# openai/baselines

Hardware: NVIDIA H100
Metric: PPO2 learner env-steps/sec (higher is better)
Workload: dtype f16 operands / f32 accumulate (GAE f64 carry)

## Files before the change

### baselines_b200/csrc/common.cuh

```cuda
#pragma once
#include <cuda.h>
#include <cuda_fp16.h>
#include <cuda_runtime.h>
#include <stdint.h>

#include "../../include/b200rl.h"

namespace b200rl {

void set_last_error(const char* fmt, ...);

inline int check_launch(const char* what) {
  cudaError_t e = cudaGetLastError();
  if (e != cudaSuccess) {
    set_last_error("%s: %s", what, cudaGetErrorString(e));
    return B200RL_ERR_CUDA;
  }
  return B200RL_OK;
}

#define B200RL_REQUIRE(cond, ...)                 \
  do {                                            \
    if (!(cond)) {                                \
      ::b200rl::set_last_error(__VA_ARGS__);      \
      return B200RL_ERR_ARG;                      \
    }                                             \
  } while (0)

__host__ __device__ inline int ceil_div(int a, int b) { return (a + b - 1) / b; }
__host__ __device__ inline long long ceil_div_ll(long long a, long long b) { return (a + b - 1) / b; }

float* det_workspace(size_t floats, cudaStream_t stream);
int sum_partials(const float* ws, int parts, long long rows, int cols, float* out, long long ldo, cudaStream_t stream);
int device_num_sms();

#ifdef __CUDACC__
__device__ __forceinline__ uint32_t smem_u32(const void* p) {
  return static_cast<uint32_t>(__cvta_generic_to_shared(p));
}

__device__ __forceinline__ void mbar_init(uint64_t* bar, uint32_t count) {
  asm volatile("mbarrier.init.shared::cta.b64 [%0], %1;" ::"r"(smem_u32(bar)), "r"(count));
}
__device__ __forceinline__ void fence_barrier_init() {
  asm volatile("fence.mbarrier_init.release.cluster;" ::: "memory");
}
__device__ __forceinline__ void fence_proxy_async_smem() {
  asm volatile("fence.proxy.async.shared::cta;" ::: "memory");
}
__device__ __forceinline__ void mbar_arrive_expect_tx(uint64_t* bar, uint32_t bytes) {
  asm volatile("mbarrier.arrive.expect_tx.shared::cta.b64 _, [%0], %1;" ::"r"(smem_u32(bar)), "r"(bytes)
               : "memory");
}
__device__ __forceinline__ void mbar_arrive(uint64_t* bar) {
  asm volatile("mbarrier.arrive.shared::cta.b64 _, [%0];" ::"r"(smem_u32(bar)) : "memory");
}
static constexpr uint32_t MBAR_SUSPEND_NS = 20000;
__device__ __forceinline__ bool mbar_try_wait(uint64_t* bar, uint32_t parity) {
  uint32_t ok;
  asm volatile(
      "{\n\t.reg .pred p;\n\t"
      "mbarrier.try_wait.parity.shared::cta.b64 p, [%1], %2, %3;\n\t"
      "selp.u32 %0, 1, 0, p;\n\t}"
      : "=r"(ok)
      : "r"(smem_u32(bar)), "r"(parity), "r"(MBAR_SUSPEND_NS)
      : "memory");
  return ok != 0;
}
__device__ __forceinline__ void mbar_wait(uint64_t* bar, uint32_t parity) {
  while (!mbar_try_wait(bar, parity)) {
  }
}

__device__ __forceinline__ uint32_t cluster_ctarank() {
  uint32_t r;
  asm volatile("mov.u32 %0, %%cluster_ctarank;" : "=r"(r));
  return r;
}
__device__ __forceinline__ uint32_t cluster_nctarank() {
  uint32_t n;
  asm volatile("mov.u32 %0, %%cluster_nctarank;" : "=r"(n));
  return n;
}
__device__ __forceinline__ void cluster_sync() {
  asm volatile("barrier.cluster.arrive.release;\n\tbarrier.cluster.wait.acquire;" ::: "memory");
// ... 62 lines not shown
```

### baselines_b200/csrc/conv_shift.cu

```cuda
#include <stdlib.h>

#include <type_traits>

#include "common.cuh"
#include "tc_common.cuh"

namespace b200rl {

static constexpr int SH_BM = 128;
static constexpr int SH_CONSUMER_WARPS = 8;
static constexpr int SH_TMA_WARP = SH_CONSUMER_WARPS;
__host__ __device__ constexpr int sh_threads(bool u8) { return (SH_CONSUMER_WARPS + 1) * 32 + (u8 ? 256 : 0); }
static constexpr int SH_MAX_TAPS = 16;
__host__ __device__ constexpr int sh_arows(int KH) { return KH == 1 ? 160 : 144; }
__host__ __device__ constexpr int sh_stages(int KH) { return KH == 1 ? 6 : 4; }
static constexpr int SH_U8_STAGES = 12;
static constexpr int SH_U8_WRES_BYTES = 16 * 1024;
__host__ __device__ constexpr int sh_wgrad_krows(bool u8) { return u8 ? 128 : 64; }
__host__ __device__ constexpr int sh_wres_bytes(int KH, bool u8) {
  return u8 ? SH_U8_WRES_BYTES : KH == 1 ? 80 * 1024 : 64 * 1024;
}
static constexpr int SH_BAR_BYTES = 512;
__host__ __device__ constexpr int sh_mask_stage_bytes(int BN, bool DACT) { return DACT ? SH_BM * BN / 8 : 0; }
static constexpr int SH_EPI_WARP_BYTES = 16 * 64;
static constexpr int SH_EPI_BYTES = SH_CONSUMER_WARPS * SH_EPI_WARP_BYTES;
static constexpr int SH_WROWS_K = 96;
static constexpr int SH_WABYTES = SH_WROWS_K * 128;
__host__ __device__ constexpr int sh_wgrad_qw(int BN, int KH, bool u8) { return u8 ? 2 : BN == 32 ? 4 : KH == 1 ? 3 : 2; }

static constexpr int SH_ORDER_BAR = 2;
__device__ __forceinline__ void order_wait(int wg) {
  asm volatile("bar.sync %0, %1;" ::"r"(SH_ORDER_BAR + wg), "n"(SH_CONSUMER_WARPS * 32) : "memory");
}
__device__ __forceinline__ void order_pass(int wg) {
  asm volatile("bar.arrive %0, %1;" ::"r"(SH_ORDER_BAR + 1 - wg), "n"(SH_CONSUMER_WARPS * 32) : "memory");
}

struct AddrMap {
  int mode;
  long long sN, sY, sX;
  int Cq, s;
  int Cq_log2, s_log2;
};

__device__ __forceinline__ long long map_rowbase(const AddrMap& a, int n, int y, int x) {
  if (a.mode == 2) {
    const int sm = a.s - 1;
    return (long long)n * a.sN + (long long)(y >> a.s_log2) * a.sY + (long long)(x >> a.s_log2) * a.sX +
           ((((y & sm) << a.s_log2) + (x & sm)) << a.Cq_log2);
  }
  if (a.mode == 1) return (long long)n * a.sN + ((long long)y << a.s_log2) * a.sY + ((long long)x << a.s_log2) * a.sX;
  return (long long)n * a.sN + (long long)y * a.sY + (long long)x * a.sX;
}
__device__ __forceinline__ long long map_coloff(const AddrMap& a, int col) {
  if (a.mode == 1) {
    const int cls = col >> a.Cq_log2;
    return (long long)(cls >> a.s_log2) * a.sY + (long long)(cls & (a.s - 1)) * a.sX + (col & (a.Cq - 1));
  }
  return col;
}

struct FastDiv {
  uint32_t mul, sh, d;
  __device__ __forceinline__ uint32_t div(uint32_t n) const { return __umulhi(n, mul) >> sh; }
};
static FastDiv make_fastdiv(uint32_t d) {
  FastDiv f;
  f.d = d;
  uint32_t s = 0;
// ... 9 lines not shown
  const long long* idx;
  long long sample_bytes;
  int row_bytes;
  int y_bytes, x_bytes;
  FastDiv per, wg;
};

static constexpr int U8_WARPS = 8;

__device__ __forceinline__ void u8x16_to_f16(const uint4& q, uint4& lo, uint4& hi) {
  const uint32_t w[4] = {q.x, q.y, q.z, q.w};
  uint32_t o[8];
  const __half2 k1024 = __floats2half2_rn(1024.0f, 1024.0f);
#pragma unroll
  for (int i = 0; i < 4; ++i) {
    const uint32_t a = __byte_perm(w[i], 0x64646464u, 0x5140);
    const uint32_t b = __byte_perm(w[i], 0x64646464u, 0x5342);
    const __half2 ha = __hsub2(*reinterpret_cast<const __half2*>(&a), k1024);
    const __half2 hb = __hsub2(*reinterpret_cast<const __half2*>(&b), k1024);
    o[2 * i] = *reinterpret_cast<const uint32_t*>(&ha);
    o[2 * i + 1] = *reinterpret_cast<const uint32_t*>(&hb);
  }
  lo = make_uint4(o[0], o[1], o[2], o[3]);
  hi = make_uint4(o[4], o[5], o[6], o[7]);
}


__device__ __forceinline__ uint4 ldg_stream_v4(const void* p) {
  uint4 v;
  asm volatile("ld.global.nc.L1::no_allocate.v4.u32 {%0,%1,%2,%3}, [%4];"
               : "=r"(v.x), "=r"(v.y), "=r"(v.z), "=r"(v.w)
               : "l"(p));
  return v;
}
__device__ __forceinline__ void st_shared_v4(uint32_t addr, const uint4& v) {
  asm volatile("st.shared.v4.b32 [%0], {%1,%2,%3,%4};" ::"r"(addr), "r"(v.x), "r"(v.y), "r"(v.z), "r"(v.w) : "memory");
}

template <int TR, int STAGES>
struct U8Ring {
  static constexpr int UPT = TR / 32;
  static constexpr int ROWS = STAGES * TR + 32;
  static constexpr int BYTES = ROWS * 128;
  static_assert(TR % 32 == 0 && BYTES % 1024 == 0, "ring keeps the 1024 B swizzle atoms aligned");
};

__device__ __forceinline__ long long u8_lookup(const U8Src& u, long long row_start, int unit, int total, long long M,
                                               int lane) {
  const long long m = row_start + (long long)unit * 32 + lane;
  if (unit >= total || m < 0 || m >= M) return -1;
  const uint32_t n = u.per.div((uint32_t)m);
  return u.idx ? __ldg(u.idx + n) : (long long)n;
}
__device__ __forceinline__ void u8_load(const U8Src& u, long long row_start, int unit, long long sb, int lane,
                                        uint4 (&q)[4]) {
  if (sb >= 0) {
    const uint32_t mm = (uint32_t)(row_start + (long long)unit * 32 + lane);
    const uint32_t rem = mm - u.per.div(mm) * u.per.d;
    const uint32_t Y = u.wg.div(rem), X = rem - Y * u.wg.d;
    const uint8_t* src = u.x + sb * u.sample_bytes + (long long)(Y * (uint32_t)u.y_bytes + X * (uint32_t)u.x_bytes);
#pragma unroll
    for (int dy = 0; dy < 4; ++dy) q[dy] = ldg_stream_v4(src + (long long)dy * u.row_bytes);
  } else {
#pragma unroll
    for (int dy = 0; dy < 4; ++dy) q[dy] = make_uint4(0u, 0u, 0u, 0u);
  }
}

template <int TR, int STAGES, int D>
// ... 38 lines not shown
        }
        fence_proxy_async_smem();
        __syncwarp();
        if (lane == 0) {
          if (tile < ntiles) mbar_arrive(&full_bar[s]);
          if (ub == 0) mbar_arrive(&head_bar[s]);
        }
        u8_load(u, row_start, uc + RND, sb[d], lane, q[d]);
        sb[d] = u8_lookup(u, row_start, uc + 2 * RND, total, M, lane);
      }
    }
  }
}

struct ShiftParams {
  U8Src u8;
  FastDiv fwg, fhg;
  long long M;
  int Hg, Wg;
  int N;
  int taps;
  int shift[SH_MAX_TAPS];
  int min_shift;
  int vy, vx;
  __half* out;
  AddrMap omap;
  uint16_t* bits_out;
  const uint16_t* saved_bits;
  const float* bias;
  int act, dact;
  float alpha;
  int num_tiles;
};

__device__ __forceinline__ void stmatrix_x4(uint32_t addr, const uint32_t (&r)[4]) {
  asm volatile("stmatrix.sync.aligned.m8n8.x4.shared.b16 [%0], {%1, %2, %3, %4};" ::"r"(addr), "r"(r[0]), "r"(r[1]),
               "r"(r[2]), "r"(r[3])
               : "memory");
}
__device__ __forceinline__ uint4 ld_shared_v4(uint32_t addr) {
  uint4 v;
  asm volatile("ld.shared.v4.b32 {%0,%1,%2,%3}, [%4];" : "=r"(v.x), "=r"(v.y), "=r"(v.z), "=r"(v.w) : "r"(addr) : "memory");
  return v;
}
__device__ __forceinline__ void st_global_v4(void* p, const uint4& v) {
  asm volatile("st.global.v4.b32 [%0], {%1,%2,%3,%4};" ::"l"(p), "r"(v.x), "r"(v.y), "r"(v.z), "r"(v.w) : "memory");
}
__device__ __forceinline__ uint32_t h2_bits(__half2 h) { return *reinterpret_cast<const uint32_t*>(&h); }
__device__ __forceinline__ uint32_t mask_pair(uint32_t b8, int k) {
  const uint32_t b = b8 >> (2 * k);
  return ((b & 1u) | ((b & 2u) << 15)) * 0xffffu;
}

template <int BN, int KH, bool DACT, bool U8>
__global__ void __launch_bounds__(sh_threads(U8), 1)
conv_shift_fwd_kernel(const __grid_constant__ CUtensorMap tmX, const __grid_constant__ CUtensorMap tmW,
                      const __grid_constant__ ShiftParams p) {
  constexpr int SH_ABYTES = sh_arows(KH) * 128;
  constexpr int STAGE_BYTES = KH * SH_ABYTES;
  constexpr int STAGES = U8 ? SH_U8_STAGES : sh_stages(KH);
  using Ring = U8Ring<SH_BM, STAGES>;
  constexpr bool PINGPONG = !(BN == 128 && !DACT);
  constexpr int MH = PINGPONG ? 2 : 1;
  static_assert(PINGPONG || !U8, "the uint8 ring's release rule assumes ping-pong");
  constexpr int A_PITCH = U8 ? SH_BM * 128 : STAGE_BYTES;
  constexpr int A_TOTAL = U8 ? Ring::BYTES : STAGES * STAGE_BYTES;
  extern __shared__ uint8_t smem_raw[];
  uint8_t* smem = reinterpret_cast<uint8_t*>((reinterpret_cast<uintptr_t>(smem_raw) + 1023) & ~uintptr_t(1023));
  uint8_t* wres = smem + A_TOTAL;
  uint64_t* bars = reinterpret_cast<uint64_t*>(wres + sh_wres_bytes(KH, U8));
  uint64_t* full_bar = bars;
  uint64_t* empty_bar = bars + STAGES;
  uint64_t* w_bar = bars + 2 * STAGES;
  uint64_t* head_bar = bars + 2 * STAGES + 1;
  static_assert((3 * STAGES + 1) * 8 <= SH_BAR_BYTES, "barrier block");
  constexpr int MASK_STAGE = sh_mask_stage_bytes(BN, DACT);
  uint8_t* smask = reinterpret_cast<uint8_t*>(bars) + SH_BAR_BYTES;
  uint8_t* sepi = smask + STAGES * MASK_STAGE;

  __shared__ float s_bias[BN];
  const int warp = threadIdx.x >> 5, lane = threadIdx.x & 31;
  constexpr int w_sub = BN * 128;
  if (threadIdx.x < BN) s_bias[threadIdx.x] = (p.bias && (int)threadIdx.x < p.N) ? p.bias[threadIdx.x] : 0.0f;
  if (threadIdx.x == 0) {
    for (int s = 0; s < STAGES; ++s) {
// ... 640 lines not shown
```

### baselines_b200/csrc/gemm_wgmma.cu

```cuda
#include <stdarg.h>
#include <stdio.h>
#include <stdlib.h>

#include <map>
#include <mutex>

#include "common.cuh"
#include "tc_common.cuh"

namespace b200rl {

static constexpr int BM = 128;
static constexpr int BK = 64;
static constexpr int MMA_K = 16;
static constexpr int CONSUMER_WARPS = 8;
static constexpr int NUM_THREADS = CONSUMER_WARPS * 32 + 32;


struct ConvCoords {
  int OW, OH;
  int stride_w, stride_h;
  int lower_w, lower_h;
  int S, taps;
};

struct ShuffleOut {
  int H, W, C, s;
};

struct GemmParams {
  int M, N, K;
  int m_tiles, n_tiles, splits, kb_per_split, kb_total;
  void* C;
  long long ldc;
  const float* bias;
  const __half* saved;
  const uint16_t* saved_bits;
  long long ld_saved;
  float alpha;
  int mode, act;
  ConvCoords cv;
  ShuffleOut sh;
  bool vec32;
  int rm_C, rm_OW, rm_Wg;
  float* ws;
};

template <int BN>
struct Cfg {
  static constexpr int A_BYTES = BM * BK * 2;
  static constexpr int B_BYTES = BN * BK * 2;
  static constexpr int STAGE_BYTES = A_BYTES + B_BYTES;
  static constexpr int STAGES_RAW = (196 * 1024) / STAGE_BYTES;
  static constexpr int STAGES = STAGES_RAW > 8 ? 8 : STAGES_RAW;
  static constexpr int SMEM_BYTES = STAGES * STAGE_BYTES + 1024  + 256 ;
};

static constexpr int BRES_STAGES = 7;
static constexpr int BRES_B_BYTES = 80 * 1024;

__device__ __forceinline__ void gemm_epi_pair(const GemmParams& p, int mode, int split, int row, int col, float v0,
                                              float v1, bool two) {
  if (mode == MODE_F32_ATOMIC) {
    if (p.ws) {
      float* w = p.ws + ((long long)split * p.M + row) * p.N + col;
      w[0] = v0;
      if (two) w[1] = v1;
      return;
    }
    float* out = reinterpret_cast<float*>(p.C) + (long long)row * p.ldc + col;
    atomicAdd(out, v0);
    if (two) atomicAdd(out + 1, v1);
    return;
  }
  if (mode == MODE_F32_STORE) {
    float* out = reinterpret_cast<float*>(p.C) + (long long)row * p.ldc + col;
    out[0] = v0 + (p.bias ? p.bias[col] : 0.0f);
    if (two) out[1] = v1 + (p.bias ? p.bias[col + 1] : 0.0f);
    return;
  }
  __half* C = reinterpret_cast<__half*>(p.C);
  if (mode == MODE_F16_SHUFFLE) {
    const int cls = col / p.sh.C, c = col % p.sh.C;
    const int j = row % p.cv.OW, t3 = row / p.cv.OW;
    const int i = t3 % p.cv.OH, n = t3 / p.cv.OH;
    const int y = p.sh.s * i + cls / p.sh.s, x = p.sh.s * j + cls % p.sh.s;
    if (y < p.sh.H && x < p.sh.W) {
      const long long o = (((long long)n * p.sh.H + y) * p.sh.W + x) * p.sh.C + c;
      if (p.saved) {
        v0 *= act_grad_from_saved(__half2float(p.saved[o]), p.act);
        v1 *= act_grad_from_saved(__half2float(p.saved[o + 1]), p.act);
      }
// ... 31 lines not shown
  } else {
    out[0] = __float2half_rn(v0);
    if (two) out[1] = __float2half_rn(v1);
  }
}

template <int BN, int CPT, bool MN_MAJOR, bool IM2COL, bool BRES, int TMODE>
__global__ void __launch_bounds__(NUM_THREADS, 1)
gemm_wgmma_kernel(const __grid_constant__ CUtensorMap tmA, const __grid_constant__ CUtensorMap tmB,
                  const GemmParams p) {
  using C_ = Cfg<BN>;
  static_assert(!BRES || (IM2COL && !MN_MAJOR), "resident weights: K-major implicit conv only");
  constexpr int STAGES = BRES ? BRES_STAGES : C_::STAGES;
  constexpr int STAGE_BYTES = BRES ? C_::A_BYTES : C_::STAGE_BYTES;
  constexpr int BROWB = MN_MAJOR ? (BN >= 64 ? 128 : BN * 2) : 0;
  constexpr uint32_t LAYOUT_B = sdesc_layout(BROWB);
  constexpr int BCHUNKS = (BN >= 64) ? BN / 64 : 1;
  constexpr int TPS = BK / CPT;
  constexpr int ROWB = CPT * 2;
  constexpr uint32_t LAYOUT_A = sdesc_layout(ROWB);
  constexpr int A_SUB = BM * ROWB;
  constexpr int B_SUB = BN * ROWB;
  constexpr int A_CHUNK = BK * ROWB;
  constexpr int MCH = BM / CPT;
  extern __shared__ uint8_t smem_raw[];
  uint8_t* smem = reinterpret_cast<uint8_t*>((reinterpret_cast<uintptr_t>(smem_raw) + 1023) & ~uintptr_t(1023));
  uint8_t* bres = smem + STAGES * STAGE_BYTES;
  constexpr int ZT_BYTES = (IM2COL && !MN_MAJOR) ? B_SUB : 0;
  uint8_t* zero_tile = bres + (BRES ? BRES_B_BYTES : 0);
  uint64_t* bars = reinterpret_cast<uint64_t*>(zero_tile + ZT_BYTES);
  uint64_t* full_bar = bars;
  uint64_t* empty_bar = bars + STAGES;
  uint64_t* bres_bar = bars + 2 * STAGES;

  const int warp = threadIdx.x >> 5;
  const int lane = threadIdx.x & 31;
  const int total_work = p.m_tiles * p.n_tiles * p.splits;

  if (threadIdx.x == 0) {
    for (int s = 0; s < STAGES; ++s) {
      mbar_init(&full_bar[s], 1);
      mbar_init(&empty_bar[s], CONSUMER_WARPS);
    }
    mbar_init(bres_bar, 1);
    fence_barrier_init();
  }
  __syncthreads();

  if (warp == CONSUMER_WARPS) {
    if (elect_one()) {
      tma_prefetch_desc(&tmA);
      tma_prefetch_desc(&tmB);
      if (BRES) {
        mbar_arrive_expect_tx(bres_bar, (uint32_t)p.cv.taps * B_SUB);
        for (int g = 0; g < p.cv.taps; ++g) tma_load_2d(bres + g * B_SUB, &tmB, bres_bar, g * CPT, 0);
      }
    }
    __syncwarp();
    int s = 0;
    uint32_t ph = 0;
    for (int work = blockIdx.x; work < total_work; work += gridDim.x) {
      const int n_tile = work % p.n_tiles;
      const int t2 = work / p.n_tiles;
      const int m_tile = t2 % p.m_tiles;
      const int split = t2 / p.m_tiles;
      const int kb0 = split * p.kb_per_split;
      const int kb1 = min(kb0 + p.kb_per_split, p.kb_total);
      int cw = 0, ch = 0, cn = 0;
      if (IM2COL && !MN_MAJOR) {
        const int m0 = m_tile * BM;
        const int q = m0 % p.cv.OW, t3 = m0 / p.cv.OW;
        cw = q * p.cv.stride_w + p.cv.lower_w;
        ch = (t3 % p.cv.OH) * p.cv.stride_h + p.cv.lower_h;
        cn = t3 / p.cv.OH;
      }
      for (int kb = kb0; kb < kb1; ++kb) {
        mbar_wait(&empty_bar[s], ph ^ 1);
        if (elect_one()) {
          uint8_t* sa = smem + s * STAGE_BYTES;
          uint8_t* sb = sa + C_::A_BYTES;
          if (!MN_MAJOR) {
            const int ntap = IM2COL ? min(TPS, p.cv.taps - kb * TPS) : TPS;
            mbar_arrive_expect_tx(&full_bar[s], (uint32_t)ntap * (A_SUB + (BRES ? 0 : B_SUB)));
#pragma unroll
            for (int t = 0; t < TPS; ++t) {
              if (t < ntap) {
                const int g = kb * TPS + t;
                if (IM2COL)
                  tma_load_im2col_4d(sa + t * A_SUB, &tmA, &full_bar[s], 0, cw, ch, cn, (uint16_t)(g % p.cv.S),
                                     (uint16_t)(g / p.cv.S));
                else
                  tma_load_2d(sa + t * A_SUB, &tmA, &full_bar[s], g * CPT, m_tile * BM);
                if (!BRES) tma_load_2d(sb + t * B_SUB, &tmB, &full_bar[s], g * CPT, n_tile * BN);
              }
            }
          } else {
            int nch = MCH;
            if (IM2COL) {
              nch = min(MCH, p.cv.taps - m_tile * MCH);
              const int k0 = kb * BK;
              const int q = k0 % p.cv.OW, t3 = k0 / p.cv.OW;
              cw = q * p.cv.stride_w + p.cv.lower_w;
              ch = (t3 % p.cv.OH) * p.cv.stride_h + p.cv.lower_h;
              cn = t3 / p.cv.OH;
            }
            mbar_arrive_expect_tx(&full_bar[s], (uint32_t)nch * A_CHUNK + C_::B_BYTES);
#pragma unroll
            for (int j = 0; j < MCH; ++j) {
              if (j < nch) {
                if (IM2COL) {
                  const int g = m_tile * MCH + j;
                  tma_load_im2col_4d(sa + j * A_CHUNK, &tmA, &full_bar[s], 0, cw, ch, cn, (uint16_t)(g % p.cv.S),
                                     (uint16_t)(g / p.cv.S));
                } else {
                  tma_load_2d(sa + j * A_CHUNK, &tmA, &full_bar[s], m_tile * BM + j * CPT, kb * BK);
                }
              }
            }
#pragma unroll
            for (int j = 0; j < BCHUNKS; ++j)
              tma_load_2d(sb + j * (BK * BROWB), &tmB, &full_bar[s], n_tile * BN + j * 64, kb * BK);
          }
        }
        __syncwarp();
        if (++s == STAGES) { s = 0; ph ^= 1; }
      }
    }
  } else {
    const int wg = warp >> 2;
    const int t = threadIdx.x & 127;
    const int mode = (TMODE >= 0) ? TMODE : p.mode;
    float acc[BN / 2];
    int s = 0;
    uint32_t ph = 0;
    if (ZT_BYTES > 0) {
      for (int i = threadIdx.x; i < ZT_BYTES / 16; i += CONSUMER_WARPS * 32)
        reinterpret_cast<uint4*>(zero_tile)[i] = make_uint4(0u, 0u, 0u, 0u);
      fence_proxy_async_smem();
      asm volatile("bar.sync 1, %0;" ::"n"(CONSUMER_WARPS * 32) : "memory");
    }
    if (BRES) mbar_wait(bres_bar, 0);
    for (int work = blockIdx.x; work < total_work; work += gridDim.x) {
      const int n_tile = work % p.n_tiles;
      const int t2 = work / p.n_tiles;
      const int m_tile = t2 % p.m_tiles;
      const int split = t2 / p.m_tiles;
      const int kb0 = split * p.kb_per_split;
      const int kb1 = min(kb0 + p.kb_per_split, p.kb_total);
      int prev = -1;
      for (int kb = kb0; kb < kb1; ++kb) {
        mbar_wait(&full_bar[s], ph);
        const uint32_t st = smem_u32(smem + s * STAGE_BYTES);
        const uint32_t b_addr = BRES ? smem_u32(bres) + (uint32_t)(kb * TPS) * B_SUB : st + C_::A_BYTES;
        wgmma_fence();
        if (!MN_MAJOR) {
          const uint32_t a_addr = st + wg * 64 * ROWB;
          const int ntap = IM2COL ? min(TPS, p.cv.taps - kb * TPS) : TPS;
#pragma unroll
// ... 164 lines not shown
  const long long n = rows * cols;
  const int lane = threadIdx.x & 31, w = threadIdx.x >> 5;
  for (long long i0 = (long long)blockIdx.x * 32; i0 < n; i0 += (long long)gridDim.x * 32) {
    const long long i = i0 + lane;
    float s = 0.0f;
    if (i < n)
      for (int q = w; q < parts; q += 8) s += ws[(long long)q * n + i];
    red[w][lane] = s;
    __syncthreads();
    if (w == 0 && i < n) {
      float t = 0.0f;
#pragma unroll
      for (int k = 0; k < 8; ++k) t += red[k][lane];
      const long long r = i / cols;
      out[r * ldo + (i - r * cols)] += t;
    }
    __syncthreads();
  }
}

int sum_partials(const float* ws, int parts, long long rows, int cols, float* out, long long ldo, cudaStream_t stream) {
  const long long n = rows * cols;
  long long blocks = (n + 31) / 32;
  if (blocks > 16LL * num_sms()) blocks = 16LL * num_sms();
  sum_partials_kernel<<<(int)blocks, 256, 0, stream>>>(ws, parts, rows, cols, out, ldo);
  return check_launch("sum_partials_kernel");
}

template <int BN, int CPT, bool MN, bool IM2COL, bool BRES = false, int TMODE = -1>
static int launch(const CUtensorMap& tmA, const CUtensorMap& tmB, const GemmParams& p, int max_ctas,
                  cudaStream_t stream) {
  using C_ = Cfg<BN>;
  constexpr int ZT = (IM2COL && !MN) ? BN * CPT * 2 : 0;
  constexpr int SMEM = (BRES ? (BRES_STAGES * C_::A_BYTES + BRES_B_BYTES + 1024 + 256) : C_::SMEM_BYTES) + ZT;
  static_assert(SMEM <= 227 * 1024, "gemm: shared memory budget");
  static bool attr_set = false;
  auto kern = gemm_wgmma_kernel<BN, CPT, MN, IM2COL, BRES, TMODE>;
  if (!attr_set) {
    cudaError_t e = cudaFuncSetAttribute(kern, cudaFuncAttributeMaxDynamicSharedMemorySize, SMEM);
    if (e != cudaSuccess) {
      set_last_error("cudaFuncSetAttribute(smem=%d): %s", SMEM, cudaGetErrorString(e));
      return B200RL_ERR_CUDA;
    }
    attr_set = true;
  }
  const int total = p.m_tiles * p.n_tiles * p.splits;
  int grid = total < num_sms() ? total : num_sms();
  if (max_ctas > 0 && grid > max_ctas) grid = max_ctas;
  kern<<<grid, NUM_THREADS, SMEM, stream>>>(tmA, tmB, p);
  return check_launch("gemm_wgmma_kernel");
}

static void fill_splits(GemmParams& p, int split_k) {
  int splits = split_k < 1 ? 1 : split_k;
  if (splits > p.kb_total) splits = p.kb_total;
  p.kb_per_split = ceil_div(p.kb_total, splits);
  p.splits = ceil_div(p.kb_total, p.kb_per_split);
}

static int gemm_dispatch(int BN, int mn_major, int mode, const CUtensorMap& tmA, const CUtensorMap& tmB,
                         const GemmParams& p, int max_ctas, cudaStream_t stream) {
  if (mn_major) {
    B200RL_REQUIRE(mode == MODE_F32_ATOMIC, "gemm: the MN-major (wgrad) layout uses the fp32 atomic epilogue");
    if (BN == 64) return launch<64, 64, true, false, false, MODE_F32_ATOMIC>(tmA, tmB, p, max_ctas, stream);
    if (BN == 256) return launch<256, 64, true, false, false, MODE_F32_ATOMIC>(tmA, tmB, p, max_ctas, stream);
    return launch<128, 64, true, false, false, MODE_F32_ATOMIC>(tmA, tmB, p, max_ctas, stream);
  }
// ... 53 lines not shown
  cudaStream_t stream = static_cast<cudaStream_t>(stream_);
  B200RL_REQUIRE(A && B && C, "gemm: null operand");
  B200RL_REQUIRE(rm_C == 0 || (rm_C % 16 == 0 && rm_OW > 0 && rm_Wg >= rm_OW && (mode == MODE_F16_ACT || mode == MODE_F16_DACT)),
                 "gemm: bad column remap");
  B200RL_REQUIRE(M > 0 && N > 0 && K > 0, "gemm: bad shape M=%d N=%d K=%d", M, N, K);
  B200RL_REQUIRE((lda % 8) == 0 && (ldb % 8) == 0, "gemm: lda/ldb must be multiples of 8 fp16 (16 B): %lld %lld", lda,
                 ldb);
  B200RL_REQUIRE((reinterpret_cast<uintptr_t>(A) & 15) == 0 && (reinterpret_cast<uintptr_t>(B) & 15) == 0,
                 "gemm: operands must be 16-byte aligned");
  B200RL_REQUIRE(mode >= 0 && mode <= 3, "gemm: bad mode %d", mode);
  B200RL_REQUIRE(mode != MODE_F16_DACT || saved != nullptr || saved_bits != nullptr,
                 "gemm: MODE_F16_DACT needs the saved activation (or its bit mask)");
  B200RL_REQUIRE(saved_bits == nullptr || (mode == MODE_F16_DACT && act == ACT_RELU && (ld_saved % 16) == 0 && (N % 16) == 0),
                 "gemm: saved_bits is a ReLU mask for MODE_F16_DACT with ld_saved and N multiples of 16");

  int BN;
  if (mn_major) BN = (N > 128 && N % 256 == 0) ? 256 : (N > 64) ? 128 : 64;
  else BN = (N > 128 && (N % 256 == 0)) ? 256 : (N > 64) ? 128 : (N > 32) ? 64 : 32;

  GemmParams p = {};
  p.M = M; p.N = N; p.K = K;
  p.m_tiles = ceil_div(M, BM);
  p.n_tiles = ceil_div(N, BN);
  p.kb_total = ceil_div(K, BK);
  B200RL_REQUIRE(split_k <= 1 || mode == MODE_F32_ATOMIC, "gemm: split_k needs the fp32 atomic epilogue");
  fill_splits(p, split_k);
  p.C = C; p.ldc = ldc; p.bias = bias; p.saved = reinterpret_cast<const __half*>(saved); p.ld_saved = ld_saved;
  p.saved_bits = reinterpret_cast<const uint16_t*>(saved_bits);
  p.alpha = alpha; p.mode = mode; p.act = act;
  p.rm_C = rm_C; p.rm_OW = rm_OW; p.rm_Wg = rm_Wg;
  p.vec32 = ((ldc & 15) == 0) && ((reinterpret_cast<uintptr_t>(C) & 31) == 0) && (rm_C == 0 || (rm_C & 15) == 0) &&
            (!saved || (((ld_saved & 15) == 0) && ((reinterpret_cast<uintptr_t>(saved) & 31) == 0)));
  B200RL_REQUIRE(saved_bits == nullptr || p.vec32, "gemm: saved_bits needs 32-byte aligned 16-column output chunks");

  CUtensorMap tmA, tmB;
  int rc;
  if (!mn_major) {
    if ((rc = make_tmap(&tmA, A, M, K, lda, BK, BM)) != 0) return rc;
    if ((rc = make_tmap(&tmB, B, N, K, ldb, BK, BN)) != 0) return rc;
  } else {
    if ((rc = make_tmap(&tmA, A, K, M, lda, 64, BK)) != 0) return rc;
    if ((rc = make_tmap(&tmB, B, K, N, ldb, 64, BK)) != 0) return rc;
  }
  if (mode == MODE_F32_ATOMIC && p.splits > 1) {
    if ((p.ws = det_workspace((size_t)p.splits * M * N, stream)) == nullptr) return B200RL_ERR_CUDA;
  }
  rc = gemm_dispatch(BN, mn_major, mode, tmA, tmB, p, max_ctas, stream);
  if (rc == B200RL_OK && p.ws) rc = sum_partials(p.ws, p.splits, M, N, reinterpret_cast<float*>(C), ldc, stream);
  return rc;
}

extern "C" int b200rl_conv_gemm(const void* x, long long B, int H, int W, int C, int R, int S, int stride_h,
                                int stride_w, int pad_h, int pad_w, int OH, int OW, const void* Wt_or_dz, long long ldb,
                                void* out, long long ldc, const float* bias, const void* saved, long long ld_saved,
                                int N, int kind, int mode, int act, float alpha, int split_k, int sh_H, int sh_W,
                                int sh_C, int sh_s, void* stream_) {
  cudaStream_t stream = static_cast<cudaStream_t>(stream_);
  B200RL_REQUIRE(x && Wt_or_dz && out && B > 0, "conv_gemm: null operand");
  B200RL_REQUIRE(C == 16 || C == 32 || C == 64, "conv_gemm: channels per tap must be 16, 32 or 64 (got %d)", C);
  B200RL_REQUIRE((reinterpret_cast<uintptr_t>(x) & 15) == 0 && (ldb % 8) == 0, "conv_gemm: alignment");
  B200RL_REQUIRE(kind == 0 || kind == 1, "conv_gemm: bad kind");
  const int taps = R * S;
  const long long rows = B * OH * OW;
  B200RL_REQUIRE(rows < (1LL << 31), "conv_gemm: too many rows");
  const int lower_w = -pad_w, lower_h = -pad_h;
  const int upper_w = (OW - 1) * stride_w + 1 + lower_w - W;
// ... 54 lines not shown
```

### baselines_b200/csrc/tc_common.cuh

```cuda
#pragma once
#include "common.cuh"
#include "wgmma.cuh"

namespace b200rl {

enum : int { MODE_F16_ACT = 0, MODE_F32_STORE = 1, MODE_F32_ATOMIC = 2, MODE_F16_DACT = 3, MODE_F16_SHUFFLE = 4 };
enum : int { ACT_NONE = 0, ACT_RELU = 1, ACT_TANH = 2 };

__host__ __device__ constexpr uint32_t sdesc_layout(int row_bytes) {
  return row_bytes == 128 ? 1u : row_bytes == 64 ? 2u : 3u;
}
__device__ __forceinline__ uint64_t make_sdesc(uint32_t saddr, uint32_t lbo_bytes, uint32_t sbo_bytes, uint32_t layout) {
  uint64_t d = 0;
  d |= (uint64_t)((saddr & 0x3FFFFu) >> 4);
  d |= (uint64_t)((lbo_bytes >> 4) & 0x3FFFu) << 16;
  d |= (uint64_t)((sbo_bytes >> 4) & 0x3FFFu) << 32;
  d |= (uint64_t)layout << 62;
  return d;
}

__device__ __forceinline__ int acc_row(int t, int e) { return 16 * (t >> 5) + ((t & 31) >> 2) + 8 * ((e >> 1) & 1); }
__device__ __forceinline__ int acc_col(int t, int e) { return 8 * (e >> 2) + 2 * (t & 3) + (e & 1); }

__device__ __forceinline__ void tma_load_im2col_4d(void* smem_dst, const CUtensorMap* tmap, uint64_t* bar, int c, int w,
                                                   int h, int n, uint16_t off_w, uint16_t off_h) {
  asm volatile(
      "cp.async.bulk.tensor.4d.shared::cluster.global.im2col.mbarrier::complete_tx::bytes"
      " [%0], [%1, {%3, %4, %5, %6}], [%2], {%7, %8};"
      ::"r"(smem_u32(smem_dst)), "l"(tmap), "r"(smem_u32(bar)), "r"(c), "r"(w), "r"(h), "r"(n), "h"(off_w), "h"(off_h)
      : "memory");
}

__device__ __forceinline__ float apply_act(float x, int act) {
  if (act == ACT_RELU) return fmaxf(x, 0.0f);
  if (act == ACT_TANH) return tanhf(x);
  return x;
}
__device__ __forceinline__ float act_grad_from_saved(float h, int act) {
  if (act == ACT_RELU) return h > 0.0f ? 1.0f : 0.0f;
  if (act == ACT_TANH) return 1.0f - h * h;
  return 1.0f;
}

int make_tmap_2d_f16(CUtensorMap* tm, const void* ptr, long long rows, long long cols, long long ld, int box_cols,
                     int box_rows);

}
```

Baseline: 1.187 million.

## Add ping-pong consumer schedule and smem-staged vectorized epilogue to WGMMA GEMM

Adds a new consumer path to the generic WGMMA GEMM for non-im2col, K-major f16/f32-store modes. In this path two warpgroups alternate whole tiles in a ping-pong order with named barriers, so one group's epilogue overlaps the other's MMAs. The epilogue goes through shared memory using stmatrix/ldmatrix to issue 16-byte vector global stores, and dact masks are prefetched into smem by the producer warp on the last k-block. Helpers from the conv kernel are moved to a shared header. The change adds shared-memory use and barrier complexity, and risks ordering bugs with the expect_tx split and the mask arrival.

```diff
diff --git a/baselines_b200/csrc/common.cuh b/baselines_b200/csrc/common.cuh
--- a/baselines_b200/csrc/common.cuh
+++ b/baselines_b200/csrc/common.cuh
@@ -51,6 +51,9 @@
 __device__ __forceinline__ void mbar_arrive_expect_tx(uint64_t* bar, uint32_t bytes) {
   asm volatile("mbarrier.arrive.expect_tx.shared::cta.b64 _, [%0], %1;" ::"r"(smem_u32(bar)), "r"(bytes)
                : "memory");
+}
+__device__ __forceinline__ void mbar_expect_tx(uint64_t* bar, uint32_t bytes) {
+  asm volatile("mbarrier.expect_tx.relaxed.cta.shared::cta.b64 [%0], %1;" ::"r"(smem_u32(bar)), "r"(bytes) : "memory");
 }
 __device__ __forceinline__ void mbar_arrive(uint64_t* bar) {
   asm volatile("mbarrier.arrive.shared::cta.b64 _, [%0];" ::"r"(smem_u32(bar)) : "memory");
diff --git a/baselines_b200/csrc/conv_shift.cu b/baselines_b200/csrc/conv_shift.cu
--- a/baselines_b200/csrc/conv_shift.cu
+++ b/baselines_b200/csrc/conv_shift.cu
@@ -27,14 +27,6 @@
 static constexpr int SH_WROWS_K = 96;
 static constexpr int SH_WABYTES = SH_WROWS_K * 128;
 __host__ __device__ constexpr int sh_wgrad_qw(int BN, int KH, bool u8) { return u8 ? 2 : BN == 32 ? 4 : KH == 1 ? 3 : 2; }
-
-static constexpr int SH_ORDER_BAR = 2;
-__device__ __forceinline__ void order_wait(int wg) {
-  asm volatile("bar.sync %0, %1;" ::"r"(SH_ORDER_BAR + wg), "n"(SH_CONSUMER_WARPS * 32) : "memory");
-}
-__device__ __forceinline__ void order_pass(int wg) {
-  asm volatile("bar.arrive %0, %1;" ::"r"(SH_ORDER_BAR + 1 - wg), "n"(SH_CONSUMER_WARPS * 32) : "memory");
-}
 
 struct AddrMap {
   int mode;
@@ -110,9 +102,6 @@
                : "=r"(v.x), "=r"(v.y), "=r"(v.z), "=r"(v.w)
                : "l"(p));
   return v;
-}
-__device__ __forceinline__ void st_shared_v4(uint32_t addr, const uint4& v) {
-  asm volatile("st.shared.v4.b32 [%0], {%1,%2,%3,%4};" ::"r"(addr), "r"(v.x), "r"(v.y), "r"(v.z), "r"(v.w) : "memory");
 }
 
 template <int TR, int STAGES>
@@ -217,25 +206,6 @@
   float alpha;
   int num_tiles;
 };
-
-__device__ __forceinline__ void stmatrix_x4(uint32_t addr, const uint32_t (&r)[4]) {
-  asm volatile("stmatrix.sync.aligned.m8n8.x4.shared.b16 [%0], {%1, %2, %3, %4};" ::"r"(addr), "r"(r[0]), "r"(r[1]),
-               "r"(r[2]), "r"(r[3])
-               : "memory");
-}
-__device__ __forceinline__ uint4 ld_shared_v4(uint32_t addr) {
-  uint4 v;
-  asm volatile("ld.shared.v4.b32 {%0,%1,%2,%3}, [%4];" : "=r"(v.x), "=r"(v.y), "=r"(v.z), "=r"(v.w) : "r"(addr) : "memory");
-  return v;
-}
-__device__ __forceinline__ void st_global_v4(void* p, const uint4& v) {
-  asm volatile("st.global.v4.b32 [%0], {%1,%2,%3,%4};" ::"l"(p), "r"(v.x), "r"(v.y), "r"(v.z), "r"(v.w) : "memory");
-}
-__device__ __forceinline__ uint32_t h2_bits(__half2 h) { return *reinterpret_cast<const uint32_t*>(&h); }
-__device__ __forceinline__ uint32_t mask_pair(uint32_t b8, int k) {
-  const uint32_t b = b8 >> (2 * k);
-  return ((b & 1u) | ((b & 2u) << 15)) * 0xffffu;
-}
 
 template <int BN, int KH, bool DACT, bool U8>
 __global__ void __launch_bounds__(sh_threads(U8), 1)
diff --git a/baselines_b200/csrc/gemm_wgmma.cu b/baselines_b200/csrc/gemm_wgmma.cu
--- a/baselines_b200/csrc/gemm_wgmma.cu
+++ b/baselines_b200/csrc/gemm_wgmma.cu
@@ -3,6 +3,7 @@
 #include <stdlib.h>
 
 #include <map>
+#include <type_traits>
 #include <mutex>
 
 #include "common.cuh"
@@ -42,6 +43,8 @@
   ConvCoords cv;
   ShuffleOut sh;
   bool vec32;
+  bool vec16;
+  bool saved16;
   int rm_C, rm_OW, rm_Wg;
   float* ws;
 };
@@ -56,8 +59,32 @@
   static constexpr int SMEM_BYTES = STAGES * STAGE_BYTES + 1024  + 256 ;
 };
 
+__host__ __device__ constexpr bool staged_epi(bool mn_major, bool im2col, int tmode) {
+  return !mn_major && !im2col && (tmode == MODE_F16_ACT || tmode == MODE_F16_DACT || tmode == MODE_F32_STORE);
+}
+static constexpr int EPI_WARP_BYTES = 16 * 64;
+__host__ __device__ constexpr int staged_mask_bytes(int BN, int tmode) { return tmode == MODE_F16_DACT ? BM * BN / 8 : 0; }
+template <int BN, int TMODE>
+__host__ __device__ constexpr int staged_smem_bytes() {
+  return Cfg<BN>::STAGES * staged_mask_bytes(BN, TMODE) + CONSUMER_WARPS * EPI_WARP_BYTES;
+}
+__host__ __device__ constexpr bool gemm_pingpong(int BN, int tmode) {
+  return BN <= 64 || (BN == 128 && tmode != MODE_F32_STORE);
+}
+
 static constexpr int BRES_STAGES = 7;
 static constexpr int BRES_B_BYTES = 80 * 1024;
+
+__device__ __forceinline__ uint4 ld_nc_v4(const void* p) {
+  uint4 v;
+  asm volatile("ld.global.nc.v4.u32 {%0,%1,%2,%3}, [%4];" : "=r"(v.x), "=r"(v.y), "=r"(v.z), "=r"(v.w) : "l"(p));
+  return v;
+}
+__device__ __forceinline__ unsigned short ld_nc_u16(const void* p) {
+  unsigned short v;
+  asm volatile("ld.global.nc.u16 %0, [%1];" : "=h"(v) : "l"(p));
+  return v;
+}
 
 __device__ __forceinline__ void gemm_epi_pair(const GemmParams& p, int mode, int split, int row, int col, float v0,
                                               float v1, bool two) {
@@ -155,6 +182,12 @@
   uint64_t* full_bar = bars;
   uint64_t* empty_bar = bars + STAGES;
   uint64_t* bres_bar = bars + 2 * STAGES;
+  constexpr bool STAGED = staged_epi(MN_MAJOR, IM2COL, TMODE);
+  constexpr bool PINGPONG = STAGED && gemm_pingpong(BN, TMODE);
+  constexpr int MASK_STAGE = STAGED ? staged_mask_bytes(BN, TMODE) : 0;
+  uint8_t* smask = reinterpret_cast<uint8_t*>(bars) + 256;
+  uint8_t* sepi = smask + STAGES * MASK_STAGE;
+  __shared__ float s_bias[2][STAGED ? BN : 1];
 
   const int warp = threadIdx.x >> 5;
   const int lane = threadIdx.x & 31;
@@ -163,7 +196,7 @@
   if (threadIdx.x == 0) {
     for (int s = 0; s < STAGES; ++s) {
       mbar_init(&full_bar[s], 1);
-      mbar_init(&empty_bar[s], CONSUMER_WARPS);
+      mbar_init(&empty_bar[s], PINGPONG ? 4 : CONSUMER_WARPS);
     }
     mbar_init(bres_bar, 1);
     fence_barrier_init();
@@ -199,12 +232,15 @@
       }
       for (int kb = kb0; kb < kb1; ++kb) {
         mbar_wait(&empty_bar[s], ph ^ 1);
+        const bool mstage = MASK_STAGE > 0 && p.saved_bits != nullptr && kb + 1 == kb1;
         if (elect_one()) {
           uint8_t* sa = smem + s * STAGE_BYTES;
           uint8_t* sb = sa + C_::A_BYTES;
           if (!MN_MAJOR) {
             const int ntap = IM2COL ? min(TPS, p.cv.taps - kb * TPS) : TPS;
-            mbar_arrive_expect_tx(&full_bar[s], (uint32_t)ntap * (A_SUB + (BRES ? 0 : B_SUB)));
+            const uint32_t tx = (uint32_t)ntap * (A_SUB + (BRES ? 0 : B_SUB));
+            if (mstage) mbar_expect_tx(&full_bar[s], tx);
+            else mbar_arrive_expect_tx(&full_bar[s], tx);
 #pragma unroll
             for (int t = 0; t < TPS; ++t) {
               if (t < ntap) {
@@ -246,7 +282,217 @@
           }
         }
         __syncwarp();
+        if (mstage) {
+          constexpr int WPR = BN / 16;
+          uint16_t* dst = reinterpret_cast<uint16_t*>(smask + s * MASK_STAGE);
+          const int m0 = m_tile * BM, w0 = n_tile * WPR, nw = p.N >> 4;
+          const long long pitch = p.ld_saved >> 4;
+#pragma unroll 4
+          for (int i = lane; i < BM * WPR; i += 32) {
+            const int r = i / WPR, j = i % WPR;
+            dst[i] = (m0 + r < p.M && w0 + j < nw) ? __ldg(p.saved_bits + (long long)(m0 + r) * pitch + w0 + j)
+                                                   : (uint16_t)0;
+          }
+          __threadfence_block();
+          __syncwarp();
+          if (lane == 0) mbar_arrive(&full_bar[s]);
+        }
         if (++s == STAGES) { s = 0; ph ^= 1; }
+      }
+    }
+  } else if constexpr (STAGED) {
+    constexpr int MH = PINGPONG ? 2 : 1;
+    const int wg = __shfl_sync(0xffffffffu, warp >> 2, 0), t = threadIdx.x & 127;
+    const int row0 = PINGPONG ? 0 : wg * 64;
+    const int kbt = p.kb_total;
+    const int tile_count =
+        (int)blockIdx.x < total_work ? (total_work - (int)blockIdx.x + (int)gridDim.x - 1) / (int)gridDim.x : 0;
+    const int er = lane & 15, ep = lane >> 4;
+    const int erow = row0 + 16 * (warp & 3) + er;
+    uint32_t epi_addr[2];
+#pragma unroll
+    for (int jj = 0; jj < 2; ++jj)
+      epi_addr[jj] = smem_u32(sepi + warp * EPI_WARP_BYTES) + er * 64 + (((2 * jj + ep) ^ ((er >> 1) & 3)) << 4);
+    const bool masked = TMODE == MODE_F16_DACT && p.saved_bits != nullptr;
+    const bool has_bias = TMODE != MODE_F16_DACT && p.bias != nullptr;
+    __half* Ch = reinterpret_cast<__half*>(p.C);
+    float acc[MH][BN / 2];
+    auto release = [&](int st) {
+      __syncwarp();
+      if (lane == 0) mbar_arrive(&empty_bar[st]);
+    };
+    for (int i = PINGPONG ? wg : 0; i < tile_count; i += PINGPONG ? 2 : 1) {
+      const int work = (int)blockIdx.x + i * (int)gridDim.x;
+      const int n_tile = work % p.n_tiles, m_tile = work / p.n_tiles;
+      const int col0 = n_tile * BN;
+      if (has_bias) {
+        asm volatile("bar.sync %0, 128;" ::"r"(4 + wg) : "memory");
+        for (int c = t; c < BN; c += 128) s_bias[wg][c] = col0 + c < p.N ? __ldg(p.bias + col0 + c) : 0.0f;
+        asm volatile("bar.sync %0, 128;" ::"r"(4 + wg) : "memory");
+      }
+      const long long q0 = (long long)i * kbt;
+      int s = (int)(q0 % STAGES);
+      uint32_t ph = (uint32_t)(q0 / STAGES) & 1u;
+      if (PINGPONG && i > 0) order_wait(wg);
+      int prev = -1;
+      for (int kb = 0; kb < kbt; ++kb) {
+        mbar_wait(&full_bar[s], ph);
+        const uint32_t st = smem_u32(smem + s * STAGE_BYTES);
+        wgmma_fence();
+#pragma unroll
+        for (int tp = 0; tp < TPS; ++tp) {
+#pragma unroll
+          for (int k = 0; k < CPT / MMA_K; ++k) {
+            const uint64_t bdesc = make_sdesc(st + C_::A_BYTES + tp * B_SUB + k * (MMA_K * 2), 16, 8 * ROWB, LAYOUT_A);
+#pragma unroll
+            for (int mh = 0; mh < MH; ++mh) {
+              const uint64_t adesc =
+                  make_sdesc(st + tp * A_SUB + (row0 + mh * 64) * ROWB + k * (MMA_K * 2), 16, 8 * ROWB, LAYOUT_A);
+              wgmma_f16<BN, 0, 0>(acc[mh], adesc, bdesc, (kb > 0 || tp > 0 || k > 0) ? 1u : 0u);
+            }
+          }
+        }
+        wgmma_commit();
+        wgmma_wait<1>();
+        if (prev >= 0) release(prev);
+        prev = s;
+        if (++s == STAGES) { s = 0; ph ^= 1; }
+      }
+      if (PINGPONG && i + 1 < tile_count) order_pass(wg);
+      wgmma_wait<0>();
+      if constexpr (TMODE == MODE_F32_STORE) {
+        release(prev);
+#pragma unroll
+        for (int mh = 0; mh < MH; ++mh) {
+          const int q = t & 3;
+          const bool odd = q & 1;
+          const int orow = m_tile * BM + row0 + mh * 64 + 16 * (warp & 3) + (lane >> 2) + (odd ? 8 : 0);
+          float* Cf = reinterpret_cast<float*>(p.C) + (long long)orow * p.ldc;
+#pragma unroll
+          for (int b = 0; b < BN / 8; ++b) {
+            const int c = 8 * b + 2 * q;
+            const float b0 = has_bias ? s_bias[wg][c] : 0.0f, b1 = has_bias ? s_bias[wg][c + 1] : 0.0f;
+            const float f0 = fmaf(acc[mh][4 * b], p.alpha, b0), f1 = fmaf(acc[mh][4 * b + 1], p.alpha, b1);
+            const float f2 = fmaf(acc[mh][4 * b + 2], p.alpha, b0), f3 = fmaf(acc[mh][4 * b + 3], p.alpha, b1);
+            const float s0 = __shfl_xor_sync(0xffffffffu, odd ? f0 : f2, 1);
+            const float s1 = __shfl_xor_sync(0xffffffffu, odd ? f1 : f3, 1);
+            const float o[4] = {odd ? s0 : f0, odd ? s1 : f1, odd ? f2 : s0, odd ? f3 : s1};
+            const int oc = col0 + 8 * b + 2 * (q & ~1);
+            if (orow < p.M && oc < p.N) {
+              if (p.vec16 && oc + 4 <= p.N) {
+                st_global_v4(Cf + oc, make_uint4(__float_as_uint(o[0]), __float_as_uint(o[1]), __float_as_uint(o[2]),
+                                                 __float_as_uint(o[3])));
+              } else {
+#pragma unroll
+                for (int k = 0; k < 4; ++k)
+                  if (oc + k < p.N) Cf[oc + k] = o[k];
+              }
+            }
+          }
+        }
+      } else {
+        auto epi16 = [&](auto masked_c) {
+        constexpr bool MASKED = decltype(masked_c)::value;
+        uint32_t mrow[MH][MASKED ? (BN + 31) / 32 : 1];
+        if constexpr (MASKED) {
+#pragma unroll
+          for (int mh = 0; mh < MH; ++mh) {
+            const uint32_t r = smem_u32(smask + prev * MASK_STAGE) + (uint32_t)((erow + mh * 64) * (BN / 8));
+#pragma unroll
+            for (int w = 0; w < BN / 32; ++w)
+              asm volatile("ld.shared.b32 %0, [%1];" : "=r"(mrow[mh][w]) : "r"(r + 4 * w));
+          }
+          __threadfence_block();
+        }
+        release(prev);
+#pragma unroll
+        for (int mh = 0; mh < MH; ++mh) {
+          const int grow = m_tile * BM + erow + mh * 64;
+          const bool rok = grow < p.M;
+#pragma unroll
+          for (int ps = 0; ps < BN / 32; ++ps) {
+#pragma unroll
+            for (int jj = 0; jj < 2; ++jj) {
+              const int b = 2 * (2 * ps + jj);
+              uint32_t hs[4];
+              if constexpr (TMODE == MODE_F16_DACT && !MASKED) {
+                const int gc = col0 + 16 * (2 * ps + jj) + 8 * ep;
+                uint4 sv = make_uint4(0u, 0u, 0u, 0u);
+                if (rok && gc < p.N) {
+                  const __half* sp = p.saved + (long long)grow * p.ld_saved + gc;
+                  if (p.saved16 && gc + 8 <= p.N) {
+                    sv = ld_nc_v4(sp);
+                  } else {
+                    uint32_t w[4] = {0u, 0u, 0u, 0u};
+#pragma unroll
+                    for (int k = 0; k < 8; ++k)
+                      if (gc + k < p.N) w[k >> 1] |= (uint32_t)ld_nc_u16(sp + k) << (16 * (k & 1));
+                    sv = make_uint4(w[0], w[1], w[2], w[3]);
+                  }
+                }
+                st_shared_v4(epi_addr[jj], sv);
+                __syncwarp();
+                ldmatrix_x4(epi_addr[jj], hs);
+                __syncwarp();
+              }
+              uint32_t r[4];
+#pragma unroll
+              for (int k = 0; k < 4; ++k) {
+                const int e = 4 * (b + (k >> 1)) + 2 * (k & 1);
+                const int c = 8 * (b + (k >> 1)) + 2 * (t & 3);
+                float v0 = __fmul_rn(acc[mh][e], p.alpha), v1 = __fmul_rn(acc[mh][e + 1], p.alpha);
+                if (TMODE == MODE_F16_ACT) {
+                  if (has_bias) {
+                    v0 = __fadd_rn(v0, s_bias[wg][c]);
+                    v1 = __fadd_rn(v1, s_bias[wg][c + 1]);
+                  }
+                  v0 = apply_act(v0, p.act);
+                  v1 = apply_act(v1, p.act);
+                } else if constexpr (!MASKED) {
+                  const __half2 h = *reinterpret_cast<const __half2*>(&hs[k]);
+                  v0 = __fmul_rn(v0, act_grad_from_saved(__low2float(h), p.act));
+                  v1 = __fmul_rn(v1, act_grad_from_saved(__high2float(h), p.act));
+                }
+                r[k] = h2_bits(__floats2half2_rn(v0, v1));
+              }
+              stmatrix_x4(epi_addr[jj], r);
+            }
+            __syncwarp();
+#pragma unroll
+            for (int jj = 0; jj < 2; ++jj) {
+              const int j = 2 * ps + jj;
+              uint4 v = ld_shared_v4(epi_addr[jj]);
+              if constexpr (MASKED) {
+                const uint32_t b8 = (mrow[mh][j >> 1] >> (16 * (j & 1) + 8 * ep)) & 0xffu;
+                v.x &= mask_pair(b8, 0);
+                v.y &= mask_pair(b8, 1);
+                v.z &= mask_pair(b8, 2);
+                v.w &= mask_pair(b8, 3);
+              }
+              const int gc = col0 + 16 * j + 8 * ep;
+              if (rok && gc < p.N) {
+                long long oc = gc;
+                if (p.rm_C > 0) {
+                  const int c16 = col0 + 16 * j, pix = c16 / p.rm_C;
+                  oc = (long long)((pix / p.rm_OW) * p.rm_Wg + pix % p.rm_OW) * p.rm_C + (c16 - pix * p.rm_C) + 8 * ep;
+                }
+                __half* out = Ch + (long long)grow * p.ldc + oc;
+                if (p.vec16 && gc + 8 <= p.N) {
+                  st_global_v4(out, v);
+                } else {
+                  const uint32_t w[4] = {v.x, v.y, v.z, v.w};
+#pragma unroll
+                  for (int k = 0; k < 8; ++k)
+                    if (gc + k < p.N) out[k] = __ushort_as_half((unsigned short)(w[k >> 1] >> (16 * (k & 1))));
+                }
+              }
+            }
+            __syncwarp();
+          }
+        }
+        };
+        if (TMODE == MODE_F16_DACT && masked) epi16(std::integral_constant<bool, TMODE == MODE_F16_DACT>{});
+        else epi16(std::false_type{});
       }
     }
   } else {
@@ -477,7 +723,8 @@
                   cudaStream_t stream) {
   using C_ = Cfg<BN>;
   constexpr int ZT = (IM2COL && !MN) ? BN * CPT * 2 : 0;
-  constexpr int SMEM = (BRES ? (BRES_STAGES * C_::A_BYTES + BRES_B_BYTES + 1024 + 256) : C_::SMEM_BYTES) + ZT;
+  constexpr int SMEM = (BRES ? (BRES_STAGES * C_::A_BYTES + BRES_B_BYTES + 1024 + 256) : C_::SMEM_BYTES) + ZT +
+                       (staged_epi(MN, IM2COL, TMODE) ? staged_smem_bytes<BN, TMODE>() : 0);
   static_assert(SMEM <= 227 * 1024, "gemm: shared memory budget");
   static bool attr_set = false;
   auto kern = gemm_wgmma_kernel<BN, CPT, MN, IM2COL, BRES, TMODE>;
@@ -597,6 +844,8 @@
   p.vec32 = ((ldc & 15) == 0) && ((reinterpret_cast<uintptr_t>(C) & 31) == 0) && (rm_C == 0 || (rm_C & 15) == 0) &&
             (!saved || (((ld_saved & 15) == 0) && ((reinterpret_cast<uintptr_t>(saved) & 31) == 0)));
   B200RL_REQUIRE(saved_bits == nullptr || p.vec32, "gemm: saved_bits needs 32-byte aligned 16-column output chunks");
+  p.vec16 = ((reinterpret_cast<uintptr_t>(C) & 15) == 0) && (ldc % (mode == MODE_F32_STORE ? 4 : 8)) == 0;
+  p.saved16 = saved && ((reinterpret_cast<uintptr_t>(saved) & 15) == 0) && (ld_saved % 8) == 0;
 
   CUtensorMap tmA, tmB;
   int rc;
diff --git a/baselines_b200/csrc/tc_common.cuh b/baselines_b200/csrc/tc_common.cuh
--- a/baselines_b200/csrc/tc_common.cuh
+++ b/baselines_b200/csrc/tc_common.cuh
@@ -42,6 +42,43 @@
   return 1.0f;
 }
 
+static constexpr int ORDER_BAR = 2;
+__device__ __forceinline__ void order_wait(int wg) {
+  asm volatile("bar.sync %0, %1;" ::"r"(ORDER_BAR + wg), "n"(256) : "memory");
+}
+__device__ __forceinline__ void order_pass(int wg) {
+  asm volatile("bar.arrive %0, %1;" ::"r"(ORDER_BAR + 1 - wg), "n"(256) : "memory");
+}
+
+__device__ __forceinline__ void stmatrix_x4(uint32_t addr, const uint32_t (&r)[4]) {
+  asm volatile("stmatrix.sync.aligned.m8n8.x4.shared.b16 [%0], {%1, %2, %3, %4};" ::"r"(addr), "r"(r[0]), "r"(r[1]),
+               "r"(r[2]), "r"(r[3])
+               : "memory");
+}
+__device__ __forceinline__ void ldmatrix_x4(uint32_t addr, uint32_t (&r)[4]) {
+  asm volatile("ldmatrix.sync.aligned.m8n8.x4.shared.b16 {%0, %1, %2, %3}, [%4];"
+               : "=r"(r[0]), "=r"(r[1]), "=r"(r[2]), "=r"(r[3])
+               : "r"(addr)
+               : "memory");
+}
+__device__ __forceinline__ void st_shared_v4(uint32_t addr, const uint4& v) {
+  asm volatile("st.shared.v4.b32 [%0], {%1,%2,%3,%4};" ::"r"(addr), "r"(v.x), "r"(v.y), "r"(v.z), "r"(v.w) : "memory");
+}
+__device__ __forceinline__ uint4 ld_shared_v4(uint32_t addr) {
+  uint4 v;
+  asm volatile("ld.shared.v4.b32 {%0,%1,%2,%3}, [%4];" : "=r"(v.x), "=r"(v.y), "=r"(v.z), "=r"(v.w) : "r"(addr) : "memory");
+  return v;
+}
+__device__ __forceinline__ void st_global_v4(void* p, const uint4& v) {
+  asm volatile("st.global.v4.b32 [%0], {%1,%2,%3,%4};" ::"l"(p), "r"(v.x), "r"(v.y), "r"(v.z), "r"(v.w) : "memory");
+}
+__device__ __forceinline__ uint32_t h2_bits(__half2 h) { return *reinterpret_cast<const uint32_t*>(&h); }
+__device__ __forceinline__ uint32_t mask_pair(uint32_t b8, int k) {
+  const uint32_t b = b8 >> (2 * k);
+  return ((b & 1u) | ((b & 2u) << 15)) * 0xffffu;
+}
+
+
 int make_tmap_2d_f16(CUtensorMap* tm, const void* ptr, long long rows, long long cols, long long ld, int box_cols,
                      int box_rows);
 
```

Measured after the change: 1.279 million (median of 6 runs). 7.7% higher.
